# steineggerlab/folddisco

Hardware: AMD Instinct MI355X
Metric: structures/sec indexed (higher is better)
Workload: dtype f32+u32; 1 GPU; Swiss-Prot scale: 542000 synthetic AFDB-shaped structures (175035960 residues, 17705019118 postings, 26085150307 value bytes) index build, PDBTrRosetta default; 1 rank(s), contiguous id ranges, per rank 1 build call(s) of <= 542000 structures: one resident index, no merge; structures=542000, structures_per_gpu=542000, residues=175035960, postings=17705019118, parallelism=shard-by-structure x1, build_calls_per_rank=1

## Files before the change

### folddisco_amd/csrc/fd_postings.h

```cpp
#pragma once
#include <hip/hip_runtime.h>
#include <stdint.h>
#include "fd_postings_host.h"

#ifndef FD_WAVE
#define FD_WAVE 64
#endif

#define FD_VALUE_SLACK 16

__host__ __device__ __forceinline__ uint32_t fd_varint_len(uint32_t v) {
#if defined(__HIP_DEVICE_COMPILE__)
    return v == 0 ? 1u : 1u + (31u - (uint32_t)__clz(v)) / 7u;
#else
    return v == 0 ? 1u : 1u + (31u - (uint32_t)__builtin_clz(v)) / 7u;
#endif
}

__host__ __device__ __forceinline__ uint64_t fd_varint_pack(uint32_t v, uint32_t len) {
    const uint32_t g = (v & 0x7fu) | (v & 0x3f80u) << 1 | (v & 0x1fc000u) << 2 | (v & 0xfe00000u) << 3;
    const uint32_t cont = (uint32_t)(0x80808080ull >> (40u - 8u * len));
    return (uint64_t)(v >> 28) << 32 | (g | cont);
}

__device__ __forceinline__ uint32_t fd_varint_at(unsigned long long w, uint32_t *nf) {
    const unsigned long long stop = ~w & 0x8080808080ull;
    const uint32_t n = (uint32_t)__ffsll((long long)stop) >> 3;
    *nf = n;
    uint32_t v = 0;
#pragma unroll
    for (uint32_t k = 0; k < 5; ++k) if (k < n) v |= (uint32_t)((w >> (8 * k)) & 0x7full) << (7 * k);
    return v;
}
__device__ __forceinline__ uint32_t fd_first_varint(const uint8_t *__restrict__ p, uint32_t *nf) {
    unsigned long long w;
    __builtin_memcpy(&w, p, 8);
    return fd_varint_at(w, nf);
}

typedef unsigned int fd_u32x4 __attribute__((ext_vector_type(4)));
__device__ __forceinline__ void fd_list_copy(uint8_t *__restrict__ d, uint32_t head, uint32_t dl, const uint8_t *__restrict__ sp, uint64_t n, uint32_t sub) {
    if (sub < dl) d[sub] = (uint8_t)(((head >> (7u * sub)) & 0x7fu) | (sub + 1u < dl ? 0x80u : 0u));
    d += dl;
    uint64_t o = (uint64_t)sub * 16u;
    for (; o + 16 <= n; o += 128) {
        fd_u32x4 v;
        __builtin_memcpy(&v, sp + o, 16);
        __builtin_memcpy(d + o, &v, 16);
    }
    if (o < n) for (uint64_t z = o; z < n; ++z) d[z] = sp[z];
}

__device__ __forceinline__ void fd_varint_store(uint8_t *o, uint32_t v, uint32_t ln) {
    for (uint32_t b = 0; b < ln; ++b) { o[b] = (uint8_t)((v & 0x7fu) | (b + 1 < ln ? 0x80u : 0u)); v >>= 7; }
}

__device__ __forceinline__ bool fd_id_local(uint32_t id, uint32_t first_id, uint64_t S, uint64_t *loc) {
    *loc = (uint64_t)id - first_id;
    return id >= first_id && *loc < S;
}

__device__ __forceinline__ uint32_t fd_wave_sum(uint32_t v) {
    for (int o = FD_WAVE / 2; o > 0; o >>= 1) v += __shfl_xor(v, o, FD_WAVE);
    return v;
}
__device__ __forceinline__ uint32_t fd_wave_max(uint32_t v) {
    for (int o = FD_WAVE / 2; o > 0; o >>= 1) { const uint32_t u = __shfl_xor(v, o, FD_WAVE); v = u > v ? u : v; }
    return v;
}
__device__ __forceinline__ uint32_t fd_wave_scan_add(uint32_t v, uint32_t lane) {
    for (int o = 1; o < FD_WAVE; o <<= 1) { const uint32_t u = __shfl_up(v, o, FD_WAVE); if ((int)lane >= o) v += u; }
    return v;
}
template <class T>
__device__ __forceinline__ T fd_wave_scan_max(T v, uint32_t lane) {
    for (int o = 1; o < FD_WAVE; o <<= 1) { const T u = __shfl_up(v, o, FD_WAVE); if ((int)lane >= o && u > v) v = u; }
    return v;
}

__device__ __forceinline__ uint32_t fd_load4(const uint8_t *p) { uint32_t w; __builtin_memcpy(&w, p, 4); return w; }
struct fd_step { uint32_t tb, sb, d[4], nf[4], dsum; unsigned long long win; };
__device__ __forceinline__ void fd_decode_step(uint32_t w, uint32_t nxt, uint64_t p, uint64_t b1, uint32_t lane, bool prev_term, fd_step *s) {
    uint32_t inm = 0, tb = 0;
#pragma unroll
    for (uint32_t j = 0; j < 4; ++j) {
        const bool in = p + j < b1;
        inm |= (in ? 1u : 0u) << j;
        tb |= (in && !((w >> (8 * j)) & 0x80u) ? 1u : 0u) << j;
    }
    const uint32_t tb_prev = __shfl_up(tb, 1, FD_WAVE);
    const uint32_t before0 = lane ? (tb_prev >> 3) & 1u : (prev_term ? 1u : 0u);
    s->tb = tb;
    s->sb = ((tb << 1) | before0) & inm & 0xfu;
    uint32_t w_hi = __shfl_down(w, 1, FD_WAVE);
    const uint32_t n0 = __shfl(nxt, 0, FD_WAVE);
    if (lane == FD_WAVE - 1) w_hi = n0;
    s->win = ((unsigned long long)w_hi << 32) | w;
    s->dsum = 0;
#pragma unroll
    for (uint32_t j = 0; j < 4; ++j) {
        uint32_t nfj = 0;
        s->d[j] = (s->sb >> j) & 1u ? fd_varint_at(s->win >> (8 * j), &nfj) : 0u;
        s->nf[j] = (s->sb >> j) & 1u ? nfj : 0u;
        s->dsum += s->d[j];
    }
}
template <class G>
__device__ __forceinline__ void fd_lane_starts(const fd_step &s, uint32_t id, G &&g) {
#pragma unroll
    for (uint32_t j = 0; j < 4; ++j)
        if ((s.sb >> j) & 1u) { id += s.d[j]; g(j, id); }
}
template <class F>
__device__ __forceinline__ void fd_wave_walk(const uint8_t *__restrict__ value, uint64_t b0, uint64_t b1, uint32_t lane, F &&f) {
    uint32_t run_id = 0;
    bool prev_term = true;
    const uint64_t p0 = b0 + 4u * lane;
    uint32_t cur = p0 < b1 ? fd_load4(value + p0) : 0u;
    for (uint64_t base = b0; base < b1; base += 4u * FD_WAVE) {
        const uint64_t p = base + 4u * lane, pn = p + 4u * FD_WAVE;
        const uint32_t nxt = pn < b1 ? fd_load4(value + pn) : 0u;
        fd_step s;
        fd_decode_step(cur, nxt, p, b1, lane, prev_term, &s);
        const uint32_t dinc = fd_wave_scan_add(s.dsum, lane);
        f(s, run_id + dinc - s.dsum);
        run_id += __shfl(dinc, FD_WAVE - 1, FD_WAVE);
        prev_term = (__shfl(s.tb, FD_WAVE - 1, FD_WAVE) >> 3) & 1u;
        cur = nxt;
    }
}
```

### folddisco_amd/csrc/k_index.hip

```cpp
#include "fd_device.h"
#include "fd_postings.h"

#define ENC_THREADS 256
#define ENC_ITEMS 8
#define ENC_TILE (ENC_THREADS * ENC_ITEMS)

struct enc_item { uint32_t len; uint32_t head; uint32_t delta; uint32_t hash; };

template <typename V> struct enc_codec;
template <> struct enc_codec<uint32_t> {
    static __device__ __forceinline__ uint32_t hash(uint32_t k) { return k; }
    static __device__ __forceinline__ uint32_t id(uint32_t, uint32_t v, uint32_t) { return v; }
};
template <> struct enc_codec<uint16_t> {
    static __device__ __forceinline__ uint32_t hash(uint32_t k) { return k >> 2; }
    static __device__ __forceinline__ uint32_t id(uint32_t k, uint16_t v, uint32_t first_id) { return first_id + (((k & 3u) << 16) | v); }
};

#define ENC_BUCKETS 40u
struct enc_b24 {
    const uint64_t *bo;
    uint32_t b0, b1;
    bool cst;
    uint32_t ev;
    __device__ __forceinline__ uint32_t at(uint64_t p) const { uint32_t b = b0; while (b < b1 && p >= bo[b + 1]) ++b; return b; }
};
struct enc_b24_raw { uint64_t o; uint32_t e0, e1; };
__device__ __forceinline__ enc_b24_raw enc_b24_fetch(const uint64_t *__restrict__ bo, const uint16_t *__restrict__ vals, uint64_t n) {
    const uint64_t t0 = (uint64_t)blockIdx.x * (256 * 8);
    const uint64_t t1 = (t0 + 256 * 8 < n ? t0 + 256 * 8 : n) - 1;
    const uint64_t tp = t0 ? t0 - 1 : 0;
    const uint32_t lane = threadIdx.x & 63;
    enc_b24_raw R;
    R.o = lane >= 1 && lane <= ENC_BUCKETS ? bo[lane] : ~0ull;
    R.e0 = vals[tp];
    R.e1 = vals[t1];
    return R;
}
__device__ __forceinline__ enc_b24 enc_b24_setup(const uint64_t *__restrict__ bo, uint64_t n, const enc_b24_raw &R) {
    const uint64_t t0 = (uint64_t)blockIdx.x * (256 * 8);
    const uint64_t t1 = (t0 + 256 * 8 < n ? t0 + 256 * 8 : n) - 1;
    const uint64_t tp = t0 ? t0 - 1 : 0;
    const uint32_t lane = threadIdx.x & 63;
    const bool in = lane >= 1 && lane <= ENC_BUCKETS;
    enc_b24 K;
    K.bo = bo;
    K.b0 = (uint32_t)__popcll(__ballot(in && R.o <= tp));
    K.b1 = (uint32_t)__popcll(__ballot(in && R.o <= t1));
    if (K.b0 >= ENC_BUCKETS) K.b0 = ENC_BUCKETS - 1;
    if (K.b1 >= ENC_BUCKETS) K.b1 = ENC_BUCKETS - 1;
    const uint32_t e0 = (uint32_t)__builtin_amdgcn_readfirstlane((int)R.e0);
    K.ev = (uint32_t)__builtin_amdgcn_readfirstlane((int)R.e1);
    K.cst = (K.b0 == K.b1) & (e0 == K.ev);
    return K;
}
__global__ void k_enc_bucket_starts(const uint64_t *__restrict__ seg_off, uint64_t S, uint64_t *__restrict__ bo) {
    if (threadIdx.x <= ENC_BUCKETS) bo[threadIdx.x] = seg_off[(uint64_t)threadIdx.x * S];
}

template <typename V, bool B24>
__device__ __forceinline__ enc_b24 enc_load_full(const uint32_t *__restrict__ keys, const V *__restrict__ ids, uint64_t n, uint64_t base,
                                                 const uint64_t *__restrict__ bo, uint32_t *k, uint32_t *v) {
    typedef unsigned int u32x4 __attribute__((ext_vector_type(4)));
    enc_b24_raw R = {};
    if (B24) R = enc_b24_fetch(bo, (const uint16_t *)ids, n);
    const u32x4 *kp = reinterpret_cast<const u32x4 *>(keys + base);
    u32x4 a = __builtin_nontemporal_load(&kp[0]), b = __builtin_nontemporal_load(&kp[1]);
    k[0] = a.x; k[1] = a.y; k[2] = a.z; k[3] = a.w; k[4] = b.x; k[5] = b.y; k[6] = b.z; k[7] = b.w;
    enc_b24 K = {};
    if (B24) K = enc_b24_setup(bo, n, R);
    if (B24 && K.cst) {
#pragma unroll
        for (int j = 0; j < ENC_ITEMS; ++j) v[j] = K.ev;
    } else if (sizeof(V) == 2) {
        u32x4 w = __builtin_nontemporal_load(reinterpret_cast<const u32x4 *>(ids + base));
        v[0] = w.x & 0xffffu; v[1] = w.x >> 16; v[2] = w.y & 0xffffu; v[3] = w.y >> 16;
        v[4] = w.z & 0xffffu; v[5] = w.z >> 16; v[6] = w.w & 0xffffu; v[7] = w.w >> 16;
    } else {
        const u32x4 *vp = reinterpret_cast<const u32x4 *>(ids + base);
        u32x4 c = __builtin_nontemporal_load(&vp[0]), d = __builtin_nontemporal_load(&vp[1]);
        v[0] = c.x; v[1] = c.y; v[2] = c.z; v[3] = c.w; v[4] = d.x; v[5] = d.y; v[6] = d.z; v[7] = d.w;
    }
    return K;
}
template <typename V, bool B24>
__device__ __forceinline__ enc_b24 enc_load_tail(const uint32_t *__restrict__ keys, const V *__restrict__ ids, uint64_t n, uint64_t base,
                                                 const uint64_t *__restrict__ bo, uint32_t *k, uint32_t *v) {
    enc_b24 K = {};
    if (B24) K = enc_b24_setup(bo, n, enc_b24_fetch(bo, (const uint16_t *)ids, n));
#pragma unroll
    for (int j = 0; j < ENC_ITEMS; ++j) {
        uint64_t p = base + j;
        k[j] = p < n ? keys[p] : 0u;
        v[j] = B24 && K.cst ? K.ev : p < n ? (uint32_t)ids[p] : 0u;
    }
    return K;
}

template <typename V, bool B24>
__device__ __forceinline__ void enc_load_classify(const uint32_t *__restrict__ keys, const V *__restrict__ ids, uint64_t n, uint64_t base,
                                                  uint32_t first_id, enc_item *it, const uint64_t *__restrict__ bo, uint32_t *pred_id = nullptr) {
    uint32_t k[ENC_ITEMS], v[ENC_ITEMS];
    const bool full = B24 ? ((uint64_t)blockIdx.x + 1) * ENC_TILE <= n : base + ENC_ITEMS <= n;
    const enc_b24 K = full ? enc_load_full<V, B24>(keys, ids, n, base, bo, k, v) : enc_load_tail<V, B24>(keys, ids, n, base, bo, k, v);
    uint32_t pk = __shfl_up(k[ENC_ITEMS - 1], 1, FD_WAVE), pv = __shfl_up(v[ENC_ITEMS - 1], 1, FD_WAVE);
    if ((threadIdx.x & 63) == 0 && base > 0 && base < n) { pk = keys[base - 1]; pv = B24 && K.cst ? K.ev : (uint32_t)ids[base - 1]; }
    uint32_t ph, pid;
    uint32_t hb[ENC_ITEMS];
    if (B24) {
        uint32_t pb = K.b0;
#pragma unroll
        for (int j = 0; j < ENC_ITEMS; ++j) hb[j] = K.b0 << 24;
        if (K.b0 != K.b1) {
            if (base) pb = K.at(base - 1);
#pragma unroll
            for (int j = 0; j < ENC_ITEMS; ++j) if (base + j < n) hb[j] = K.at(base + j) << 24;
        }
        ph = pb << 24 | pv << 8 | pk >> 24; pid = first_id + (pk & 0xffffffu);
    } else { ph = enc_codec<V>::hash(pk); pid = enc_codec<V>::id(pk, (V)pv, first_id); }
    if (pred_id) *pred_id = pid;
    bool have_prev = base > 0;
#pragma unroll
    for (int j = 0; j < ENC_ITEMS; ++j) {
        uint64_t p = base + j;
        uint32_t h, id;
        if (B24) { h = hb[j] | v[j] << 8 | k[j] >> 24; id = first_id + (k[j] & 0xffffffu); }
        else { h = enc_codec<V>::hash(k[j]); id = enc_codec<V>::id(k[j], (V)v[j], first_id); }
        bool in = p < n;
        bool head = !have_prev || ph != h;
        bool dup = !head && pid == id;
        it[j].hash = h;
        it[j].head = (in && head) ? 1u : 0u;
        it[j].delta = head ? id : id - pid;
        it[j].len = (!in || dup) ? 0u : fd_varint_len(it[j].delta);
        ph = h; pid = id; have_prev = true;
    }
}

__device__ __forceinline__ uint64_t wave_incl_scan64(uint64_t v) {
    uint32_t lane = threadIdx.x & 63;
    for (int off = 1; off < 64; off <<= 1) {
        uint64_t t = __shfl_up(v, off, FD_WAVE);
        if ((int)lane >= off) v += t;
    }
    return v;
}
__device__ __forceinline__ uint64_t block_excl_scan_packed(uint64_t v, uint64_t *sm, uint64_t *total) {
    uint32_t lane = threadIdx.x & 63, wid = threadIdx.x >> 6;
    uint64_t inc = wave_incl_scan64(v);
    if (lane == 63) sm[wid] = inc;
    __syncthreads();
    uint64_t base = 0, tot = 0;
#pragma unroll
    for (uint32_t w = 0; w < ENC_THREADS / 64; ++w) {
        uint64_t t = sm[w];
        if (w < wid) base += t;
        tot += t;
    }
    __syncthreads();
    *total = tot;
    return inc - v + base;
}

template <typename V, bool B24>
__global__ __launch_bounds__(ENC_THREADS) void k_enc_sizes(const uint32_t *__restrict__ keys, const V *__restrict__ ids, uint64_t n, uint32_t first_id,
                                                           uint32_t *__restrict__ tile_bytes, uint32_t *__restrict__ tile_heads,
                                                           uint32_t *__restrict__ tile_posts, const uint64_t *__restrict__ bo) {
    __shared__ uint64_t sm[ENC_THREADS / 64];
    uint64_t base = (uint64_t)blockIdx.x * ENC_TILE + (uint64_t)threadIdx.x * ENC_ITEMS;
    uint32_t bytes = 0, heads = 0, posts = 0;
    enc_item it[ENC_ITEMS];
    enc_load_classify<V, B24>(keys, ids, n, base, first_id, it, bo);
#pragma unroll
    for (int k = 0; k < ENC_ITEMS; ++k) {
        bytes += it[k].len;
        heads += it[k].head;
        posts += it[k].len ? 1u : 0u;
    }
    uint64_t tot;
    block_excl_scan_packed(((uint64_t)bytes << 32) | heads, sm, &tot);
    uint32_t pw = posts;
    for (int off = 32; off > 0; off >>= 1) pw += __shfl_down(pw, off, FD_WAVE);
    __shared__ uint32_t pp[ENC_THREADS / 64];
    if ((threadIdx.x & 63) == 0) pp[threadIdx.x >> 6] = pw;
    __syncthreads();
    if (threadIdx.x == 0) {
        tile_bytes[blockIdx.x] = (uint32_t)(tot >> 32);
        tile_heads[blockIdx.x] = (uint32_t)tot;
        uint32_t t = 0;
        for (int w = 0; w < ENC_THREADS / 64; ++w) t += pp[w];
        tile_posts[blockIdx.x] = t;
    }
}

#define ENC_LDS_BYTES (ENC_TILE * 5 + 32)
static_assert(ENC_LDS_BYTES % 16 == 0 && (ENC_TILE * 5 + 15 + 15) / 16 * 16 <= ENC_LDS_BYTES, "s_bytes: a full tile of five-byte varints must fit");
template <typename V, bool B24>
__global__ __launch_bounds__(ENC_THREADS) void k_enc_write(const uint32_t *__restrict__ keys, const V *__restrict__ ids, uint64_t n, uint32_t first_id,
                                                           const uint64_t *__restrict__ tile_byte_off, const uint64_t *__restrict__ tile_head_off,
                                                           uint8_t *__restrict__ value, uint32_t *__restrict__ hashes, uint64_t *__restrict__ offsets,
                                                           uint32_t *__restrict__ last_ids, const uint64_t *__restrict__ bo) {
    typedef unsigned int u32x4 __attribute__((ext_vector_type(4)));
    __shared__ uint64_t sm[ENC_THREADS / 64];
    __shared__ __attribute__((aligned(16))) uint8_t s_bytes[ENC_LDS_BYTES];
    uint32_t *const s_dw = reinterpret_cast<uint32_t *>(s_bytes);
    const uint64_t base = (uint64_t)blockIdx.x * ENC_TILE + (uint64_t)threadIdx.x * ENC_ITEMS;
    enc_item it[ENC_ITEMS];
    uint32_t bytes = 0, heads = 0;
    uint32_t run_id = 0;
    enc_load_classify<V, B24>(keys, ids, n, base, first_id, it, bo, &run_id);
#pragma unroll
    for (int k = 0; k < ENC_ITEMS; ++k) { bytes += it[k].len; heads += it[k].head; }
    const uint64_t mine = ((uint64_t)bytes << 32) | heads;
    const uint64_t inc = wave_incl_scan64(mine);
    if ((threadIdx.x & 63) == 63) sm[threadIdx.x >> 6] = inc;
    const uint64_t tile_b0 = tile_byte_off[blockIdx.x];
    const uint32_t shift = (uint32_t)(tile_b0 & 15ull);
    __syncthreads();
    uint64_t ex = inc - mine, tot = 0;
#pragma unroll
    for (uint32_t w = 0; w < ENC_THREADS / 64; ++w) {
        const uint64_t t = sm[w];
        if (w < (threadIdx.x >> 6)) ex += t;
        tot += t;
    }
    const uint32_t tile_len = (uint32_t)(tot >> 32);
    const uint32_t end = shift + tile_len;
    for (uint32_t c = threadIdx.x * 16; c < end; c += ENC_THREADS * 16) *reinterpret_cast<u32x4 *>(s_bytes + c) = u32x4{0u, 0u, 0u, 0u};
    __syncthreads();
    const uint32_t lo = shift + (uint32_t)(ex >> 32);
    const bool tail = base < n && n - base <= ENC_ITEMS;
    if (heads | (tail ? 1u : 0u)) {
        uint64_t hoff = tile_head_off[blockIdx.x] + (uint32_t)ex;
        const uint64_t boff = tile_b0 + (ex >> 32);
        const uint32_t k_last = tail ? (uint32_t)(n - base) - 1u : ENC_ITEMS;
        uint32_t pre = 0;
#pragma unroll
        for (uint32_t k = 0; k < ENC_ITEMS; ++k) {
            if (it[k].head) {
                hashes[hoff] = it[k].hash;
                offsets[hoff] = boff + pre;
                if (hoff) last_ids[hoff - 1] = run_id;
                ++hoff;
            }
            run_id = it[k].head ? it[k].delta : run_id + it[k].delta;
            if (k == k_last) last_ids[hoff - 1] = run_id;
            pre += it[k].len;
        }
    }
    uint32_t pos = lo;
    uint64_t acc = 0;
#pragma unroll
    for (int k = 0; k < ENC_ITEMS; ++k) {
        const uint32_t len = it[k].len;
        acc |= fd_varint_pack(len ? it[k].delta : 0u, len) << (8u * (pos & 3u));
        atomicOr(&s_dw[pos >> 2], (uint32_t)acc);
        const uint32_t npos = pos + len;
        const uint32_t filled = (npos >> 2) - (pos >> 2);
        if (filled > 1) { atomicOr(&s_dw[(pos >> 2) + 1], (uint32_t)(acc >> 32)); acc = 0; }
        else acc = filled ? acc >> 32 : acc;
        pos = npos;
    }
    atomicOr(&s_dw[pos >> 2], (uint32_t)acc);
    __syncthreads();
    uint8_t *gbase = value + (tile_b0 - shift);
    for (uint32_t c = threadIdx.x * 16; c < end; c += ENC_THREADS * 16) {
        if (c >= shift && c + 16 <= end) {
            *reinterpret_cast<u32x4 *>(gbase + c) = *reinterpret_cast<const u32x4 *>(s_bytes + c);
        } else {
            for (uint32_t b = c < shift ? shift : c; b < c + 16 && b < end; ++b) gbase[b] = s_bytes[b];
        }
    }
}

__global__ void k_set_u64(uint64_t *dst, uint64_t idx, const uint64_t *src) { dst[idx] = src[0]; }

uint32_t fd_enc_num_tiles(uint64_t n) { return (uint32_t)((n + ENC_TILE - 1) / ENC_TILE); }
void fd_launch_enc_sizes(const uint32_t *keys, const void *ids, int codec, uint32_t first_id, uint64_t n, uint32_t *tb, uint32_t *th, uint32_t *tp,
                         const uint64_t *seg_off, uint64_t S, uint64_t *bo, hipStream_t st) {
    if (!n) return;
    const dim3 g(fd_enc_num_tiles(n)), t(ENC_THREADS);
    if (codec == 2) hipLaunchKernelGGL(k_enc_bucket_starts, dim3(1), dim3(64), 0, st, seg_off, S, bo);
    if (codec == 2) hipLaunchKernelGGL((k_enc_sizes<uint16_t, true>), g, t, 0, st, keys, (const uint16_t *)ids, n, first_id, tb, th, tp, bo);
    else if (codec == 1) hipLaunchKernelGGL((k_enc_sizes<uint16_t, false>), g, t, 0, st, keys, (const uint16_t *)ids, n, first_id, tb, th, tp, bo);
    else hipLaunchKernelGGL((k_enc_sizes<uint32_t, false>), g, t, 0, st, keys, (const uint32_t *)ids, n, first_id, tb, th, tp, bo);
}
void fd_launch_enc_write(const uint32_t *keys, const void *ids, int codec, uint32_t first_id, uint64_t n, const uint64_t *tbo, const uint64_t *tho,
                         uint8_t *value, uint32_t *hashes, uint64_t *offsets, uint32_t *last_ids, const uint64_t *total_bytes_dev, uint64_t H,
                         const uint64_t *bo, hipStream_t st) {
    if (n) {
        const dim3 g(fd_enc_num_tiles(n)), t(ENC_THREADS);
        if (codec == 2) hipLaunchKernelGGL((k_enc_write<uint16_t, true>), g, t, 0, st, keys, (const uint16_t *)ids, n, first_id, tbo, tho, value, hashes, offsets, last_ids, bo);
        else if (codec == 1) hipLaunchKernelGGL((k_enc_write<uint16_t, false>), g, t, 0, st, keys, (const uint16_t *)ids, n, first_id, tbo, tho, value, hashes, offsets, last_ids, bo);
        else hipLaunchKernelGGL((k_enc_write<uint32_t, false>), g, t, 0, st, keys, (const uint32_t *)ids, n, first_id, tbo, tho, value, hashes, offsets, last_ids, bo);
    }
    hipLaunchKernelGGL(k_set_u64, dim3(1), dim3(1), 0, st, offsets, H, total_bytes_dev);
}
```

Baseline: 1.664 million structures/s.

## Add fast classify path for constant-bucket tiles and packed 32-bit DPP scans

Adds a specialised classification path for tiles whose ids are constant within a single bucket. It derives deltas directly from key differences, with a wave-level ballot to skip head detection when no hash boundary occurs. The count kernel takes an early-exit path that computes tile totals with a DPP wave scan instead of the general block scan. The encode kernel packs bytes and heads into one u32 and scans with DPP instead of a 64-bit shuffle scan, and skips head emission for head-free tiles. These changes add correctness risk around tile boundaries, block 0, and the 16-bit packing limits.

```diff
diff --git a/folddisco_amd/csrc/fd_postings.h b/folddisco_amd/csrc/fd_postings.h
--- a/folddisco_amd/csrc/fd_postings.h
+++ b/folddisco_amd/csrc/fd_postings.h
@@ -21,6 +21,31 @@
     const uint32_t g = (v & 0x7fu) | (v & 0x3f80u) << 1 | (v & 0x1fc000u) << 2 | (v & 0xfe00000u) << 3;
     const uint32_t cont = (uint32_t)(0x80808080ull >> (40u - 8u * len));
     return (uint64_t)(v >> 28) << 32 | (g | cont);
+}
+
+__host__ __device__ __forceinline__ bool fd_const_is_head(uint32_t k, uint32_t pk) { return ((k ^ pk) >> 24) != 0; }
+__host__ __device__ __forceinline__ uint32_t fd_delta_len(uint32_t d) {
+#if defined(__HIP_DEVICE_COMPILE__)
+    const uint32_t z = (uint32_t)__clz((int)(d << 1 | 1u));
+#else
+    const uint32_t z = (uint32_t)__builtin_clz(d << 1 | 1u);
+#endif
+    return (37u - z) * 37u >> 8;
+}
+__host__ __device__ __forceinline__ uint32_t fd_const_delta(uint32_t k, uint32_t pk, uint32_t *len) {
+    const uint32_t d = k - pk;
+    *len = fd_delta_len(d);
+    return d;
+}
+__host__ __device__ __forceinline__ uint32_t fd_const_head(uint32_t k, uint32_t first_id, uint32_t *len) {
+    const uint32_t id = first_id + (k & 0xffffffu);
+    *len = fd_varint_len(id);
+    return id;
+}
+__host__ __device__ __forceinline__ bool fd_const_classify(uint32_t k, uint32_t pk, uint32_t first_id, uint32_t *value, uint32_t *len) {
+    const bool head = fd_const_is_head(k, pk);
+    *value = head ? fd_const_head(k, first_id, len) : fd_const_delta(k, pk, len);
+    return head;
 }
 
 __device__ __forceinline__ uint32_t fd_varint_at(unsigned long long w, uint32_t *nf) {
diff --git a/folddisco_amd/csrc/k_index.hip b/folddisco_amd/csrc/k_index.hip
--- a/folddisco_amd/csrc/k_index.hip
+++ b/folddisco_amd/csrc/k_index.hip
@@ -23,10 +23,11 @@
     uint32_t b0, b1;
     bool cst;
     uint32_t ev;
+    uint32_t wpk;
     __device__ __forceinline__ uint32_t at(uint64_t p) const { uint32_t b = b0; while (b < b1 && p >= bo[b + 1]) ++b; return b; }
 };
-struct enc_b24_raw { uint64_t o; uint32_t e0, e1; };
-__device__ __forceinline__ enc_b24_raw enc_b24_fetch(const uint64_t *__restrict__ bo, const uint16_t *__restrict__ vals, uint64_t n) {
+struct enc_b24_raw { uint64_t o; uint32_t e0, e1, wpk; };
+__device__ __forceinline__ enc_b24_raw enc_b24_fetch(const uint32_t *__restrict__ keys, const uint64_t *__restrict__ bo, const uint16_t *__restrict__ vals, uint64_t n, bool full) {
     const uint64_t t0 = (uint64_t)blockIdx.x * (256 * 8);
     const uint64_t t1 = (t0 + 256 * 8 < n ? t0 + 256 * 8 : n) - 1;
     const uint64_t tp = t0 ? t0 - 1 : 0;
@@ -35,6 +36,9 @@
     R.o = lane >= 1 && lane <= ENC_BUCKETS ? bo[lane] : ~0ull;
     R.e0 = vals[tp];
     R.e1 = vals[t1];
+    const uint64_t w0 = t0 + (uint32_t)__builtin_amdgcn_readfirstlane((int)(threadIdx.x >> 6)) * (64u * 8u);
+    const uint64_t wq = full || w0 < n ? w0 : n;
+    R.wpk = keys[wq ? wq - 1 : 0];
     return R;
 }
 __device__ __forceinline__ enc_b24 enc_b24_setup(const uint64_t *__restrict__ bo, uint64_t n, const enc_b24_raw &R) {
@@ -52,6 +56,7 @@
     const uint32_t e0 = (uint32_t)__builtin_amdgcn_readfirstlane((int)R.e0);
     K.ev = (uint32_t)__builtin_amdgcn_readfirstlane((int)R.e1);
     K.cst = (K.b0 == K.b1) & (e0 == K.ev);
+    K.wpk = R.wpk;
     return K;
 }
 __global__ void k_enc_bucket_starts(const uint64_t *__restrict__ seg_off, uint64_t S, uint64_t *__restrict__ bo) {
@@ -63,15 +68,13 @@
                                                  const uint64_t *__restrict__ bo, uint32_t *k, uint32_t *v) {
     typedef unsigned int u32x4 __attribute__((ext_vector_type(4)));
     enc_b24_raw R = {};
-    if (B24) R = enc_b24_fetch(bo, (const uint16_t *)ids, n);
+    if (B24) R = enc_b24_fetch(keys, bo, (const uint16_t *)ids, n, true);
     const u32x4 *kp = reinterpret_cast<const u32x4 *>(keys + base);
     u32x4 a = __builtin_nontemporal_load(&kp[0]), b = __builtin_nontemporal_load(&kp[1]);
     k[0] = a.x; k[1] = a.y; k[2] = a.z; k[3] = a.w; k[4] = b.x; k[5] = b.y; k[6] = b.z; k[7] = b.w;
     enc_b24 K = {};
     if (B24) K = enc_b24_setup(bo, n, R);
     if (B24 && K.cst) {
-#pragma unroll
-        for (int j = 0; j < ENC_ITEMS; ++j) v[j] = K.ev;
     } else if (sizeof(V) == 2) {
         u32x4 w = __builtin_nontemporal_load(reinterpret_cast<const u32x4 *>(ids + base));
         v[0] = w.x & 0xffffu; v[1] = w.x >> 16; v[2] = w.y & 0xffffu; v[3] = w.y >> 16;
@@ -87,7 +90,7 @@
 __device__ __forceinline__ enc_b24 enc_load_tail(const uint32_t *__restrict__ keys, const V *__restrict__ ids, uint64_t n, uint64_t base,
                                                  const uint64_t *__restrict__ bo, uint32_t *k, uint32_t *v) {
     enc_b24 K = {};
-    if (B24) K = enc_b24_setup(bo, n, enc_b24_fetch(bo, (const uint16_t *)ids, n));
+    if (B24) K = enc_b24_setup(bo, n, enc_b24_fetch(keys, bo, (const uint16_t *)ids, n, false));
 #pragma unroll
     for (int j = 0; j < ENC_ITEMS; ++j) {
         uint64_t p = base + j;
@@ -97,14 +100,59 @@
     return K;
 }
 
-template <typename V, bool B24>
-__device__ __forceinline__ void enc_load_classify(const uint32_t *__restrict__ keys, const V *__restrict__ ids, uint64_t n, uint64_t base,
-                                                  uint32_t first_id, enc_item *it, const uint64_t *__restrict__ bo, uint32_t *pred_id = nullptr) {
+enum { ENC_GENERAL = 0, ENC_FAST = 1, ENC_FAST_HEADS = 2 };
+__device__ __forceinline__ int enc_classify_const(uint64_t n, uint32_t first_id, const enc_b24 &K,
+                                                  const uint32_t *k, enc_item *it, uint32_t *bytes, uint32_t *heads, uint32_t *pred_id) {
+    const uint32_t pk0 = (uint32_t)__builtin_amdgcn_update_dpp((int)K.wpk, (int)k[ENC_ITEMS - 1], 0x138, 0xf, 0xf, false);
+    uint32_t pk = pk0, hx = 0;
+#pragma unroll
+    for (int j = 0; j < ENC_ITEMS; ++j) {
+        hx |= k[j] ^ pk;
+        it[j].delta = fd_const_delta(k[j], pk, &it[j].len);
+        it[j].head = 0u; it[j].hash = 0u;
+        pk = k[j];
+    }
+    int path = ENC_FAST;
+    *heads = 0u;
+    const bool ends_stream = ((uint64_t)blockIdx.x + 1) * ENC_TILE == n;
+    if (__ballot((hx >> 24) != 0u) != 0ull || ends_stream) {
+        path = ENC_FAST_HEADS;
+        const uint32_t hash_hi = K.b0 << 24 | K.ev << 8;
+        uint32_t nh = 0;
+        pk = pk0;
+#pragma unroll
+        for (int j = 0; j < ENC_ITEMS; ++j) {
+            if (fd_const_is_head(k[j], pk)) {
+                it[j].delta = fd_const_head(k[j], first_id, &it[j].len);
+                it[j].head = 1u; it[j].hash = hash_hi | k[j] >> 24;
+                ++nh;
+            }
+            pk = k[j];
+        }
+        *heads = nh;
+        if (pred_id) *pred_id = first_id + (pk0 & 0xffffffu);
+    }
+    uint32_t b = 0;
+#pragma unroll
+    for (int j = 0; j < ENC_ITEMS; ++j) b += it[j].len;
+    *bytes = b;
+    return path;
+}
+
+template <typename V, bool B24>
+__device__ __forceinline__ int enc_load_classify(const uint32_t *__restrict__ keys, const V *__restrict__ ids, uint64_t n, uint64_t base,
+                                                 uint32_t first_id, enc_item *it, const uint64_t *__restrict__ bo, uint32_t *bytes, uint32_t *heads,
+                                                 uint32_t *pred_id = nullptr) {
     uint32_t k[ENC_ITEMS], v[ENC_ITEMS];
     const bool full = B24 ? ((uint64_t)blockIdx.x + 1) * ENC_TILE <= n : base + ENC_ITEMS <= n;
     const enc_b24 K = full ? enc_load_full<V, B24>(keys, ids, n, base, bo, k, v) : enc_load_tail<V, B24>(keys, ids, n, base, bo, k, v);
+    if (B24 && full && K.cst && blockIdx.x != 0) return enc_classify_const(n, first_id, K, k, it, bytes, heads, pred_id);
+    if (B24 && full && K.cst) {
+#pragma unroll
+        for (int j = 0; j < ENC_ITEMS; ++j) v[j] = K.ev;
+    }
     uint32_t pk = __shfl_up(k[ENC_ITEMS - 1], 1, FD_WAVE), pv = __shfl_up(v[ENC_ITEMS - 1], 1, FD_WAVE);
-    if ((threadIdx.x & 63) == 0 && base > 0 && base < n) { pk = keys[base - 1]; pv = B24 && K.cst ? K.ev : (uint32_t)ids[base - 1]; }
+    if ((threadIdx.x & 63) == 0 && base > 0 && base < n) { pk = B24 ? K.wpk : keys[base - 1]; pv = B24 && K.cst ? K.ev : (uint32_t)ids[base - 1]; }
     uint32_t ph, pid;
     uint32_t hb[ENC_ITEMS];
     if (B24) {
@@ -120,6 +168,7 @@
     } else { ph = enc_codec<V>::hash(pk); pid = enc_codec<V>::id(pk, (V)pv, first_id); }
     if (pred_id) *pred_id = pid;
     bool have_prev = base > 0;
+    uint32_t b = 0, nh = 0;
 #pragma unroll
     for (int j = 0; j < ENC_ITEMS; ++j) {
         uint64_t p = base + j;
@@ -131,12 +180,24 @@
         bool dup = !head && pid == id;
         it[j].hash = h;
         it[j].head = (in && head) ? 1u : 0u;
-        it[j].delta = head ? id : id - pid;
+        it[j].delta = !in ? 0u : head ? id : id - pid;
         it[j].len = (!in || dup) ? 0u : fd_varint_len(it[j].delta);
+        b += it[j].len; nh += it[j].head;
         ph = h; pid = id; have_prev = true;
     }
-}
-
+    *bytes = b; *heads = nh;
+    return ENC_GENERAL;
+}
+
+__device__ __forceinline__ uint32_t enc_wave_incl(uint32_t v) {
+    v += (uint32_t)__builtin_amdgcn_update_dpp(0, (int)v, 0x111, 0xf, 0xf, false);
+    v += (uint32_t)__builtin_amdgcn_update_dpp(0, (int)v, 0x112, 0xf, 0xf, false);
+    v += (uint32_t)__builtin_amdgcn_update_dpp(0, (int)v, 0x114, 0xf, 0xf, false);
+    v += (uint32_t)__builtin_amdgcn_update_dpp(0, (int)v, 0x118, 0xf, 0xf, false);
+    v += (uint32_t)__builtin_amdgcn_update_dpp(0, (int)v, 0x142, 0xa, 0xf, false);
+    v += (uint32_t)__builtin_amdgcn_update_dpp(0, (int)v, 0x143, 0xc, 0xf, false);
+    return v;
+}
 __device__ __forceinline__ uint64_t wave_incl_scan64(uint64_t v) {
     uint32_t lane = threadIdx.x & 63;
     for (int off = 1; off < 64; off <<= 1) {
@@ -170,13 +231,28 @@
     uint64_t base = (uint64_t)blockIdx.x * ENC_TILE + (uint64_t)threadIdx.x * ENC_ITEMS;
     uint32_t bytes = 0, heads = 0, posts = 0;
     enc_item it[ENC_ITEMS];
-    enc_load_classify<V, B24>(keys, ids, n, base, first_id, it, bo);
-#pragma unroll
-    for (int k = 0; k < ENC_ITEMS; ++k) {
-        bytes += it[k].len;
-        heads += it[k].head;
-        posts += it[k].len ? 1u : 0u;
-    }
+    const int path = enc_load_classify<V, B24>(keys, ids, n, base, first_id, it, bo, &bytes, &heads);
+    if (B24 && path != ENC_GENERAL) {
+        __shared__ uint32_t sw[ENC_THREADS / 64][3];
+        uint32_t wp = 0;
+#pragma unroll
+        for (int k = 0; k < ENC_ITEMS; ++k) wp += (uint32_t)__popcll(__ballot(it[k].len != 0u));
+        const uint32_t mine = bytes << 16 | heads;
+        const uint32_t wbh = (uint32_t)__builtin_amdgcn_readlane((int)enc_wave_incl(mine), 63);
+        const uint32_t wb = wbh >> 16, wh = wbh & 0xffffu;
+        if ((threadIdx.x & 63) == 0) { uint32_t *w = sw[threadIdx.x >> 6]; w[0] = wb; w[1] = wh; w[2] = wp; }
+        __syncthreads();
+        if (threadIdx.x == 0) {
+            uint32_t t[3] = {0u, 0u, 0u};
+            for (int w = 0; w < ENC_THREADS / 64; ++w) for (int q = 0; q < 3; ++q) t[q] += sw[w][q];
+            tile_bytes[blockIdx.x] = t[0];
+            tile_heads[blockIdx.x] = t[1];
+            tile_posts[blockIdx.x] = t[2];
+        }
+        return;
+    }
+#pragma unroll
+    for (int k = 0; k < ENC_ITEMS; ++k) posts += it[k].len ? 1u : 0u;
     uint64_t tot;
     block_excl_scan_packed(((uint64_t)bytes << 32) | heads, sm, &tot);
     uint32_t pw = posts;
@@ -201,51 +277,52 @@
                                                            uint8_t *__restrict__ value, uint32_t *__restrict__ hashes, uint64_t *__restrict__ offsets,
                                                            uint32_t *__restrict__ last_ids, const uint64_t *__restrict__ bo) {
     typedef unsigned int u32x4 __attribute__((ext_vector_type(4)));
-    __shared__ uint64_t sm[ENC_THREADS / 64];
+    __shared__ uint32_t sm[ENC_THREADS / 64];
     __shared__ __attribute__((aligned(16))) uint8_t s_bytes[ENC_LDS_BYTES];
     uint32_t *const s_dw = reinterpret_cast<uint32_t *>(s_bytes);
     const uint64_t base = (uint64_t)blockIdx.x * ENC_TILE + (uint64_t)threadIdx.x * ENC_ITEMS;
     enc_item it[ENC_ITEMS];
     uint32_t bytes = 0, heads = 0;
     uint32_t run_id = 0;
-    enc_load_classify<V, B24>(keys, ids, n, base, first_id, it, bo, &run_id);
-#pragma unroll
-    for (int k = 0; k < ENC_ITEMS; ++k) { bytes += it[k].len; heads += it[k].head; }
-    const uint64_t mine = ((uint64_t)bytes << 32) | heads;
-    const uint64_t inc = wave_incl_scan64(mine);
+    const int path = enc_load_classify<V, B24>(keys, ids, n, base, first_id, it, bo, &bytes, &heads, &run_id);
+    static_assert(ENC_TILE * 5 < (1 << 16), "bytes and heads of a tile are scanned as the halves of one u32");
+    const uint32_t mine = bytes << 16 | heads;
+    const uint32_t inc = enc_wave_incl(mine);
     if ((threadIdx.x & 63) == 63) sm[threadIdx.x >> 6] = inc;
     const uint64_t tile_b0 = tile_byte_off[blockIdx.x];
     const uint32_t shift = (uint32_t)(tile_b0 & 15ull);
     __syncthreads();
-    uint64_t ex = inc - mine, tot = 0;
+    uint32_t ex = inc - mine, tot = 0;
 #pragma unroll
     for (uint32_t w = 0; w < ENC_THREADS / 64; ++w) {
-        const uint64_t t = sm[w];
+        const uint32_t t = sm[w];
         if (w < (threadIdx.x >> 6)) ex += t;
         tot += t;
     }
-    const uint32_t tile_len = (uint32_t)(tot >> 32);
+    const uint32_t tile_len = tot >> 16;
     const uint32_t end = shift + tile_len;
     for (uint32_t c = threadIdx.x * 16; c < end; c += ENC_THREADS * 16) *reinterpret_cast<u32x4 *>(s_bytes + c) = u32x4{0u, 0u, 0u, 0u};
     __syncthreads();
-    const uint32_t lo = shift + (uint32_t)(ex >> 32);
-    const bool tail = base < n && n - base <= ENC_ITEMS;
-    if (heads | (tail ? 1u : 0u)) {
-        uint64_t hoff = tile_head_off[blockIdx.x] + (uint32_t)ex;
-        const uint64_t boff = tile_b0 + (ex >> 32);
-        const uint32_t k_last = tail ? (uint32_t)(n - base) - 1u : ENC_ITEMS;
-        uint32_t pre = 0;
-#pragma unroll
-        for (uint32_t k = 0; k < ENC_ITEMS; ++k) {
-            if (it[k].head) {
-                hashes[hoff] = it[k].hash;
-                offsets[hoff] = boff + pre;
-                if (hoff) last_ids[hoff - 1] = run_id;
-                ++hoff;
+    const uint32_t lo = shift + (ex >> 16);
+    if (path != ENC_FAST) {
+        const bool tail = base < n && n - base <= ENC_ITEMS;
+        if (heads | (tail ? 1u : 0u)) {
+            uint64_t hoff = tile_head_off[blockIdx.x] + (ex & 0xffffu);
+            const uint64_t boff = tile_b0 + (ex >> 16);
+            const uint32_t k_last = tail ? (uint32_t)(n - base) - 1u : ENC_ITEMS;
+            uint32_t pre = 0;
+#pragma unroll
+            for (uint32_t k = 0; k < ENC_ITEMS; ++k) {
+                if (it[k].head) {
+                    hashes[hoff] = it[k].hash;
+                    offsets[hoff] = boff + pre;
+                    if (hoff) last_ids[hoff - 1] = run_id;
+                    ++hoff;
+                }
+                run_id = it[k].head ? it[k].delta : run_id + it[k].delta;
+                if (k == k_last) last_ids[hoff - 1] = run_id;
+                pre += it[k].len;
             }
-            run_id = it[k].head ? it[k].delta : run_id + it[k].delta;
-            if (k == k_last) last_ids[hoff - 1] = run_id;
-            pre += it[k].len;
         }
     }
     uint32_t pos = lo;
@@ -253,7 +330,7 @@
 #pragma unroll
     for (int k = 0; k < ENC_ITEMS; ++k) {
         const uint32_t len = it[k].len;
-        acc |= fd_varint_pack(len ? it[k].delta : 0u, len) << (8u * (pos & 3u));
+        acc |= fd_varint_pack(it[k].delta, len) << (8u * (pos & 3u));
         atomicOr(&s_dw[pos >> 2], (uint32_t)acc);
         const uint32_t npos = pos + len;
         const uint32_t filled = (npos >> 2) - (pos >> 2);
```

Result: faster. 1.716 million structures/s, median of 6 (+3.1%).
